# yugabyte/yugabyte-db

Measured on NVIDIA H100. Metric: compaction GB/s (input bytes merged), higher is better.
Workload: dtype u8

## Files before the change

yugabyte-db_b200/csrc/engine.cu:

```cuda
#include "engine.h"
#include "host_sst.h"

#include <cuda_runtime.h>
#include <algorithm>
#include <cstdio>
#include <cstring>
#include <chrono>
#include <cstdlib>
#include <mutex>

namespace ybgpu {

#define CUDA_TRY(expr)                                                                      \
  do {                                                                                      \
    cudaError_t _e = (expr);                                                                \
    if (_e != cudaSuccess) {                                                                \
      return FailCuda(#expr, _e);                                                           \
    }                                                                                       \
  } while (0)

struct RunView {
  const uint8_t* data;
  const uint64_t* blk_off;
  const uint32_t* blk_size;
// ... 423 lines not shown
      const uint8_t* prec = srec - static_cast<size_t>(prm->M) * S;
      inside = rec_ulen(prec, S) >= static_cast<uint32_t>(g) && common_prefix_len(srec, g, prec, g) >= static_cast<uint32_t>(g) &&
               group_prefix_len(prec, rec_ulen(prec, S), prm->R.enabled != 0) == g;
    }
    if (r2 == 0) P.smode[s] = inside ? 1 : 0;
    const RunView& q = P.runs[r2];
    uint32_t lo = 0, hi = q.n_entries;
    if (pass == 1) {
      const uint32_t c0 = s_local - s_local % SAMPLE_COARSE, c1 = c0 + SAMPLE_COARSE;
      lo = P.pos[static_cast<size_t>(P.sample_base[r] + c0) * k + r2];
      if (P.sample_base[r] + c1 < P.sample_base[r + 1]) hi = P.pos[static_cast<size_t>(P.sample_base[r] + c1) * k + r2];
    }
    if (inside) {
      if (r2 == static_cast<uint32_t>(r)) lo = hi = idx;
      while (lo < hi) {
        const uint32_t mid = (lo + hi) >> 1;
        const int c = cmp_records(q.rec + static_cast<size_t>(mid) * S, srec, S);
        if (r2 < static_cast<uint32_t>(r) ? c <= 0 : c < 0) lo = mid + 1; else hi = mid;
      }
    } else {
      while (lo < hi) {
        uint32_t mid = (lo + hi) >> 1;
        const uint8_t* c = q.rec + static_cast<size_t>(mid) * S;
        if (cmp_prefix_vs_key(srec, g, c, rec_ulen(c, S)) > 0) lo = mid + 1; else hi = mid;
      }
    }
    P.pos[static_cast<size_t>(s) * k + r2] = lo;
  }
}

__global__ void __launch_bounds__(256) k_sample_bucket(PartView P, const JobParams* prm) {
  const int k = prm->k;
  for (uint32_t s = blockIdx.x * blockDim.x + threadIdx.x; s < P.n_samples; s += gridDim.x * blockDim.x) {
    unsigned long long rank = 0;
    for (int r = 0; r < k; r++) rank += P.pos[static_cast<size_t>(s) * k + r];
    if (rank == 0) continue;
    uint32_t b = static_cast<uint32_t>(rank / prm->H);
    atomicMin(&P.bucket_min[b], (rank << 28) | s);
  }
}

__device__ __forceinline__ uint32_t block_exclusive_scan(uint32_t v, uint32_t* warp_sums, uint32_t* total) {
  const int lane = threadIdx.x & 31, wid = threadIdx.x >> 5;
  uint32_t x = v;
  for (int o = 1; o < 32; o <<= 1) { uint32_t y = __shfl_up_sync(0xffffffffu, x, o); if (lane >= o) x += y; }
  __syncthreads();
  if (lane == 31) warp_sums[wid] = x;
  __syncthreads();
  if (wid == 0) {
    uint32_t w = lane < (blockDim.x >> 5) ? warp_sums[lane] : 0;
    for (int o = 1; o < 32; o <<= 1) { uint32_t y = __shfl_up_sync(0xffffffffu, w, o); if (lane >= o) w += y; }
    warp_sums[lane] = w;
  }
  __syncthreads();
  uint32_t excl = (wid ? warp_sums[wid - 1] : 0) + x - v;
  if (total) *total = warp_sums[(blockDim.x >> 5) - 1];
  return excl;
}

constexpr int TILE_CHUNK = 2048;
__global__ void __launch_bounds__(256) k_bucket_counts(PartView P, uint32_t* partial) {
  __shared__ uint32_t sh;
  if (threadIdx.x == 0) sh = 0;
  __syncthreads();
  const uint64_t base = static_cast<uint64_t>(blockIdx.x) * TILE_CHUNK;
  uint32_t c = 0;
  for (uint32_t j = threadIdx.x; j < TILE_CHUNK; j += 256) { const uint64_t i = base + j; if (i < P.n_buckets && P.bucket_min[i] != ~0ull) c++; }
  c = __reduce_add_sync(0xffffffffu, c);
  if ((threadIdx.x & 31) == 0 && c) atomicAdd(&sh, c);
  __syncthreads();
  if (threadIdx.x == 0) partial[blockIdx.x] = sh;
}
__global__ void __launch_bounds__(256) k_build_tiles(PartView P, const JobParams* prm, const uint32_t* partial , const uint32_t* total,
                                                     uint32_t* tile_lo, unsigned long long* tile_rank, JobDev* J) {
  __shared__ uint32_t warp_sums[32];
  const int k = prm->k;
  if (blockIdx.x == 0) {
    if (threadIdx.x < k) tile_lo[threadIdx.x] = 0;
    if (threadIdx.x == 0) { tile_rank[0] = 0; J->n_tiles = *total + 1; }
  }
  const uint64_t base = static_cast<uint64_t>(blockIdx.x) * TILE_CHUNK;
  constexpr int PER = TILE_CHUNK / 256;
  unsigned long long v[PER];
  uint32_t c = 0;
  for (int j = 0; j < PER; j++) { const uint64_t i = base + threadIdx.x * PER + j; v[j] = i < P.n_buckets ? P.bucket_min[i] : ~0ull; c += v[j] != ~0ull; }
  uint32_t t = 1 + partial[blockIdx.x] + block_exclusive_scan(c, warp_sums, nullptr);
  for (int j = 0; j < PER; j++) {
    if (v[j] == ~0ull) continue;
    const uint32_t s = static_cast<uint32_t>(v[j] & ((1u << 28) - 1));
    for (int r = 0; r < k; r++) tile_lo[static_cast<size_t>(t) * k + r] = P.pos[static_cast<size_t>(s) * k + r];
    tile_rank[t] = (v[j] >> 28) | (P.smode[s] ? TILE_CONT : 0ull);
    t++;
  }
}

__global__ void __launch_bounds__(256) k_tile_check(const RunView* runs, const uint32_t* tile_lo, int k, JobDev* J) {
  const uint32_t n_tiles = J->n_tiles;
  uint32_t mx = 0;
  for (uint32_t t = blockIdx.x * blockDim.x + threadIdx.x; t < n_tiles; t += gridDim.x * blockDim.x) {
    uint32_t sz = 0;
    for (int r = 0; r < k; r++) {
      const uint32_t lo = tile_lo[static_cast<size_t>(t) * k + r];
      const uint32_t hi = (t + 1 < n_tiles) ? tile_lo[static_cast<size_t>(t + 1) * k + r] : runs[r].n_entries;
      sz += hi - lo;
    }
    mx = max(mx, sz);
  }
  mx = __reduce_max_sync(0xffffffffu, mx);
  if ((threadIdx.x & 31) == 0 && mx) atomicMax(&J->max_tile, mx);
}

struct MergeView {
  const RunView* runs;
  const uint32_t* tile_lo;
  const unsigned long long* tile_rank;
  Desc* desc;
  ValueRewrite* rewrites;
  uint32_t rewrite_cap;
  uint32_t n_tiles;
  uint16_t* fk16;
  uint32_t* fkh;
  int32_t S, k;
  uint32_t cap;
};

constexpr int MERGE_THREADS = 256;
constexpr uint8_t ENT_GROUP_START = 128;
constexpr uint32_t RW_PRE_DROPPED = 0xfffffffeu;
constexpr int RANK_C = 8;
constexpr int RANK_KMAX = 16;

namespace tile_layout {
constexpr uint32_t SEG_LO = 0;
constexpr uint32_t SEG_START = SEG_LO + 4 * MAX_RUNS;
constexpr uint32_t CBASE = SEG_START + 4 * (MAX_RUNS + 2);
constexpr uint32_t CRANK = CBASE + 4 * (MAX_RUNS + 2);
constexpr uint32_t CRANK_FIXED = 2 * (RANK_KMAX + 1) * RANK_KMAX;
constexpr uint32_t CRANK_PER = 2 * RANK_KMAX / RANK_C;
constexpr uint32_t A0 = (CRANK + CRANK_FIXED + 15) & ~15u;
constexpr uint32_t ORDER_K = CRANK_PER;
constexpr uint32_t GLEN_K = ORDER_K + 2;
constexpr uint32_t GSTART_K = GLEN_K + 2;
constexpr uint32_t A1 = A0 + 16;
constexpr uint32_t PVIS_K = GSTART_K + 2;
constexpr uint32_t RES_K = PVIS_K + 2;
constexpr uint32_t RW_K = RES_K + 1;
constexpr uint32_t PFX_K = RW_K + 4;
constexpr uint32_t PFX2_K = PFX_K + 8;
constexpr uint32_t RECS_K = PFX2_K + 8;
static_assert(RANK_KMAX % RANK_C == 0 && (PFX_K % 1) == 0, "layout");
__host__ __device__ constexpr uint32_t bytes(uint32_t S, uint32_t cap) { return A1 + (RECS_K + S + 8) * cap; }
}


static_assert(MAX_RUNS <= REPLAY_MAX_RUNS, "a replay's cursors cover every run of a job");

__device__ __noinline__ int seed_continuation(FeedState* st, const JobParams* prm, const RunView* runs, const uint32_t* seg_lo, int k, int S,
                                              const uint8_t* k0_smem) {
  ReplayRun rr[REPLAY_MAX_RUNS];
  for (int r = 0; r < k; r++) { rr[r].rec = runs[r].rec; rr[r].limit = seg_lo[r]; rr[r].data = runs[r].data; rr[r].val_off = runs[r].val_off; }
  return replay_ancestors(st, prm->R, rr, k, S, k0_smem, rec_ulen(k0_smem, S), prm->bottommost, prm->last_sequence);
}

__device__ __forceinline__ int table_id_len(const uint8_t* e, uint32_t ulen) {
  return (e[0] == 'y' || e[0] == '0') ? dockey_id_size(e, ulen) : 0;
}

__device__ __noinline__ int seed_table_from_runs(Overwrite* ow0, const JobParams* prm, const RunView* runs, const uint32_t* seg_lo,
                                                 const uint32_t* seg_start, int k, int S, const uint8_t* row, int id, bool through_tile) {
  ReplayRun rr[REPLAY_MAX_RUNS];
  for (int r = 0; r < k; r++) {
    rr[r].rec = runs[r].rec; rr[r].data = runs[r].data; rr[r].val_off = runs[r].val_off;
    rr[r].limit = seg_lo[r] + (through_tile ? seg_start[r + 1] - seg_start[r] : 0u);
  }
  FeedState st;
  const int d = replay_table_seed(&st, prm->R, rr, k, S, row, static_cast<uint32_t>(id), prm->bottommost, prm->last_sequence);
  if (d < 0) return d;
  if (!st.n_ow) return 0;
  *ow0 = st.ow[0];
  return 1;
}

__device__ __noinline__ int seed_table_in_tile(FeedState* st, const JobParams* prm, const RunView* runs, const uint8_t* recs, int SS, int S,
                                               const uint16_t* order, const uint32_t* seg_lo, const uint32_t* seg_start,
                                               uint32_t i0, uint32_t i1, const uint8_t* row, int id) {
  feed_state_reset(st);
  const uint8_t* prev = nullptr;
  for (uint32_t i = i0; i < i1; i++) {
    const uint32_t li = order[i];
    const uint8_t* c = recs + static_cast<size_t>(SS) * li;
    if (rec_flags(c, S) & REC_F_HT_FILTERED) continue;
    const uint8_t* val = nullptr;
    if (rec_vlen(c, S) && has_control_fields(rec_vfirst(c, S))) {
      int r = 0;
      while (seg_start[r + 1] <= li) r++;
      val = runs[r].data + runs[r].val_off[seg_lo[r] + (li - seg_start[r])];
    }
    const int d = replay_entry(st, prm->R, c, S, val, &prev, prm->bottommost, prm->last_sequence);
    if (d < 0) return d;
  }
  table_seed(st, row, static_cast<uint32_t>(id));
  return 0;
}

__device__ __forceinline__ uint32_t block_exclusive_max(uint32_t v, uint32_t* warp_sums) {
  const int lane = threadIdx.x & 31, wid = threadIdx.x >> 5;
  uint32_t x = v;
  for (int o = 1; o < 32; o <<= 1) { const uint32_t y = __shfl_up_sync(0xffffffffu, x, o); if (lane >= o) x = max(x, y); }
  uint32_t ex = __shfl_up_sync(0xffffffffu, x, 1);
  if (lane == 0) ex = 0;
  __syncthreads();
  if (lane == 31) warp_sums[wid] = x;
  __syncthreads();
  if (wid == 0) {
    uint32_t m = lane < (blockDim.x >> 5) ? warp_sums[lane] : 0;
    for (int o = 1; o < 32; o <<= 1) { const uint32_t y = __shfl_up_sync(0xffffffffu, m, o); if (lane >= o) m = max(m, y); }
    warp_sums[lane] = m;
  }
  __syncthreads();
  return max(wid ? warp_sums[wid - 1] : 0u, ex);
}

__global__ void __launch_bounds__(MERGE_THREADS, 3) k_merge_filter(MergeView V, const JobParams* prm, JobDev* J) {
  extern __shared__ __align__(16) uint8_t smem[];
  const int S = V.S, k = V.k;
  const int SS = S + 8;
  const uint32_t cap = V.cap;
  namespace L = tile_layout;
  uint32_t* seg_lo = reinterpret_cast<uint32_t*>(smem + L::SEG_LO);
  uint32_t* seg_start = reinterpret_cast<uint32_t*>(smem + L::SEG_START);
  uint32_t* cbase = reinterpret_cast<uint32_t*>(smem + L::CBASE);
  uint16_t* crank = reinterpret_cast<uint16_t*>(smem + L::CRANK);
  uint16_t* order = reinterpret_cast<uint16_t*>(smem + L::A0 + L::ORDER_K * cap);
  uint16_t* glen = reinterpret_cast<uint16_t*>(smem + L::A0 + L::GLEN_K * cap);
  uint16_t* gstart = reinterpret_cast<uint16_t*>(smem + L::A0 + L::GSTART_K * cap);
  uint16_t* pvis = reinterpret_cast<uint16_t*>(smem + L::A1 + L::PVIS_K * cap);
  uint8_t* res = smem + L::A1 + L::RES_K * cap;
  uint32_t* rw_slot = reinterpret_cast<uint32_t*>(smem + L::A1 + L::RW_K * cap);
  unsigned long long* pfx = reinterpret_cast<unsigned long long*>(smem + L::A1 + L::PFX_K * cap);
  unsigned long long* pfx2 = reinterpret_cast<unsigned long long*>(smem + L::A1 + L::PFX2_K * cap);
  uint8_t* recs = smem + L::A1 + L::RECS_K * cap;
  __shared__ uint32_t warp_sums[32];
  __shared__ uint32_t sh_T, sh_ngroups, sh_any_filtered, sh_any_id;
  __shared__ int sh_err;
  __shared__ uint32_t sh_c0;
  __shared__ Overwrite sh_ow0;
  __shared__ int sh_ow0_state;
  __shared__ unsigned long long sh_stats[9];
  __shared__ const uint8_t* sh_pred;
  __shared__ uint32_t sh_rb[2][MAX_RUNS + 2];

  const uint32_t tile = blockIdx.x;
  const bool cont = (V.tile_rank[tile] & TILE_CONT) != 0;
  if (threadIdx.x < 9) sh_stats[threadIdx.x] = 0;
  if (threadIdx.x < 32) {
    static_assert(MAX_RUNS <= 64, "two rounds of 32 lanes cover the runs");
    uint32_t acc = 0;
    for (int r0 = 0; r0 < k; r0 += 32) {
      const int r = r0 + static_cast<int>(threadIdx.x);
      uint32_t lo = 0, n = 0;
      if (r < k) {
        lo = V.tile_lo[static_cast<size_t>(tile) * k + r];
        const uint32_t hi = (tile + 1 < V.n_tiles) ? V.tile_lo[static_cast<size_t>(tile + 1) * k + r] : V.runs[r].n_entries;
        n = hi - lo;
      }
      uint32_t x = n;
      for (int o = 1; o < 32; o <<= 1) { const uint32_t y = __shfl_up_sync(0xffffffffu, x, o); if (static_cast<int>(threadIdx.x) >= o) x += y; }
      if (r < k) { seg_lo[r] = lo; seg_start[r] = acc + x - n; }
      acc += __shfl_sync(0xffffffffu, x, 31);
    }
    if (threadIdx.x == 0) {
      seg_start[k] = acc;
      sh_T = acc;
      sh_any_filtered = 0;
      sh_any_id = 0;
      sh_err = *reinterpret_cast<volatile int*>(&J->error);
    }
  }
  __syncthreads();
  const uint32_t T = sh_T;
  if (T == 0) return;
  if (cont && threadIdx.x == 0) atomicAdd(&J->n_cont_tiles, 1u);
  if (T > cap) { if (threadIdx.x == 0) dev_fail(J, DEV_ERR_TILE_OVERFLOW, tile); return; }

  {
    const uint32_t vpr = S >> 4;
    const uint32_t nvec = T * vpr;
    const bool vpr_pow2 = (vpr & (vpr - 1)) == 0;
    const uint32_t vpr_shift = 31 - __clz(vpr);
#pragma unroll 4
    for (uint32_t i = threadIdx.x; i < nvec; i += blockDim.x) {
      const uint32_t li = vpr_pow2 ? i >> vpr_shift : i / vpr, q = i - li * vpr;
      int r = 0;
      while (seg_start[r + 1] <= li) r++;
      const uint4 v = __ldg(reinterpret_cast<const uint4*>(V.runs[r].rec + static_cast<size_t>(seg_lo[r] + (li - seg_start[r])) * S) + q);
      uint2* d = reinterpret_cast<uint2*>(recs + static_cast<size_t>(li) * SS + 16 * q);
      d[0] = make_uint2(v.x, v.y); d[1] = make_uint2(v.z, v.w);
    }
  }
  __syncthreads();

  if (threadIdx.x < 32) {
    const uint8_t* ref = recs;
    const uint32_t ref_len = rec_ulen(ref, S);
    uint32_t c = 0xffffffffu;
    for (int r = static_cast<int>(threadIdx.x); r < k; r += 32) {
      const uint32_t n = seg_start[r + 1] - seg_start[r];
      if (!n) continue;
      const uint8_t* f = recs + static_cast<size_t>(SS) * seg_start[r];
      const uint8_t* l = recs + static_cast<size_t>(SS) * (seg_start[r + 1] - 1);
      c = min(c, min(common_prefix_len(ref, ref_len, f, rec_ulen(f, S)), common_prefix_len(ref, ref_len, l, rec_ulen(l, S))));
    }
    c = __reduce_min_sync(0xffffffffu, c);
    c = min(c, ref_len) & ~7u;
    if (c + 16 > static_cast<uint32_t>(S - 16)) c = (S - 16 >= 16) ? static_cast<uint32_t>(S - 32) & ~7u : 0;
    if (threadIdx.x == 0) sh_c0 = c;
  }
  if (threadIdx.x == 0) {
    const uint8_t* pred = nullptr;
    if (cont) {
      for (int r = 0; r < k; r++) {
        uint32_t j = seg_lo[r];
        const uint8_t* c2 = nullptr;
        while (j > 0) {
          const uint8_t* q = V.runs[r].rec + static_cast<size_t>(j - 1) * S;
          if (!(rec_flags(q, S) & REC_F_INVISIBLE)) { c2 = q; break; }
          j--;
        }
        if (c2 && (!pred || cmp_records(c2, pred, S) >= 0)) pred = c2;
      }
    }
    sh_pred = pred;
  }
  __syncthreads();
  {
    const uint32_t c0 = sh_c0;
    for (uint32_t li = threadIdx.x; li < T; li += blockDim.x)
    {
      pfx[li] = bswap64(ld_u64_aligned(recs + static_cast<size_t>(SS) * li + c0));
      pfx2[li] = bswap64(ld_u64_aligned(recs + static_cast<size_t>(SS) * li + c0 + 8));
    }
  }
  __syncthreads();

  {
    constexpr int MT = 2;
    uint16_t* bufs[2] = {order, reinterpret_cast<uint16_t*>(crank)};
    auto le = [&](uint32_t a, uint32_t b) -> bool {
      const unsigned long long pa = pfx[a], pb = pfx[b];
      if (pa != pb) return pa < pb;
      const unsigned long long qa = pfx2[a], qb = pfx2[b];
      if (qa != qb) return qa < qb;
      return cmp_records(recs + static_cast<size_t>(SS) * a, recs + static_cast<size_t>(SS) * b, S) <= 0;
    };
    for (uint32_t li = threadIdx.x; li < T; li += blockDim.x) bufs[0][li] = static_cast<uint16_t>(li);
    if (threadIdx.x <= static_cast<uint32_t>(k)) sh_rb[0][threadIdx.x] = seg_start[threadIdx.x];
    __syncthreads();
    int nruns = k, cur = 0;
    while (nruns > 1) {
      const uint16_t* src = bufs[cur]; uint16_t* dst = bufs[cur ^ 1];
      const uint32_t* rb = sh_rb[cur];
      const int npairs = (nruns + 1) >> 1;
      for (uint32_t o0 = threadIdx.x * MT; o0 < T; o0 += blockDim.x * MT) {
        int p = 0;
        while (p + 1 < npairs && rb[2 * (p + 1)] <= o0) p++;
        uint32_t a0 = rb[2 * p], a1 = rb[min(2 * p + 1, nruns)], b1 = rb[min(2 * p + 2, nruns)];
        const uint32_t d = o0 - a0, la = a1 - a0, lb = b1 - a1;
        uint32_t lo = d > lb ? d - lb : 0, hi = min(d, la);
        while (lo < hi) {
          const uint32_t mid = (lo + hi) >> 1;
          if (le(src[a0 + mid], src[a1 + (d - 1 - mid)])) lo = mid + 1; else hi = mid;
        }
        uint32_t i = a0 + lo, j = a1 + (d - lo);
        const uint32_t o_end = min(o0 + MT, T);
        for (uint32_t o = o0; o < o_end; o++) {
          while (o == b1 && p + 1 < npairs) {
            p++;
            a0 = rb[2 * p]; a1 = rb[min(2 * p + 1, nruns)]; b1 = rb[min(2 * p + 2, nruns)];
            i = a0; j = a1;
          }
          uint16_t pick;
          if (i < a1 && (j >= b1 || le(src[i], src[j]))) pick = src[i++]; else pick = src[j++];
          dst[o] = pick;
        }
      }
      if (threadIdx.x <= static_cast<uint32_t>(npairs)) sh_rb[cur ^ 1][threadIdx.x] = rb[min(2 * static_cast<int>(threadIdx.x), nruns)];
      __syncthreads();
      nruns = npairs; cur ^= 1;
    }
    if (cur) {
      for (uint32_t li = threadIdx.x; li < T; li += blockDim.x) order[li] = bufs[1][li];
    }
  }
  for (uint32_t li = threadIdx.x; li < T; li += blockDim.x) {
    int r = 0;
    while (seg_start[r + 1] <= li) r++;
    const uint32_t p = li - seg_start[r];
    const uint8_t* e = recs + static_cast<size_t>(SS) * li;
    if (p > 0 && cmp_records(e - SS, e, S) >= 0) { dev_fail(J, DEV_ERR_UNSORTED, tile); sh_err = 1; }
    int fk = 0;
    const int g = group_prefix_len(e, rec_ulen(e, S), prm->R.enabled != 0, V.fk16 ? &fk : nullptr);
    if (g < 0) { dev_fail(J, -g, tile); sh_err = 1; glen[li] = 0; } else glen[li] = static_cast<uint16_t>(g);
    if (V.fk16) {
      const uint32_t gid = V.runs[r].gid_base + seg_lo[r] + p;
      V.fk16[gid] = static_cast<uint16_t>(g < 0 ? 0 : fk);
      if (V.fkh) V.fkh[gid] = (g < 0 || fk <= 0) ? 0u : leveldb_hash(e, static_cast<uint32_t>(fk), kBloomSeed);
    }
    if (rec_flags(e, S) & REC_F_INVISIBLE) sh_any_filtered = 1;
    if (e[0] == 'y' || e[0] == '0') sh_any_id = 1;
  }
  __syncthreads();
  if (sh_err) return;

  if (sh_any_filtered) {
    if (threadIdx.x == 0) {
      uint32_t last = 0xffff;
      for (uint32_t i = 0; i < T; i++) {
        pvis[i] = static_cast<uint16_t>(last);
        if (!(rec_flags(recs + static_cast<size_t>(SS) * (order[i]), S) & REC_F_INVISIBLE)) last = i;
      }
    }
  } else {
    for (uint32_t i = threadIdx.x; i < T; i += blockDim.x) pvis[i] = static_cast<uint16_t>(i ? i - 1 : 0xffff);
  }
  __syncthreads();

  const uint32_t items = (T + blockDim.x - 1) / blockDim.x;
  uint32_t my_groups = 0;
  unsigned long long st_counted = 0, st_hidden = 0, st_obsolete = 0, st_in_k = 0, st_in_v = 0;
  for (uint32_t j = 0; j < items; j++) {
    const uint32_t i = threadIdx.x * items + j;
    if (i >= T) break;
    const uint32_t li = order[i];
    const uint8_t* e = recs + static_cast<size_t>(SS) * (li);
    uint8_t f = 0;
    if (!(rec_flags(e, S) & REC_F_INVISIBLE)) {
      f |= ENT_COUNTED; st_counted++;
      st_in_k += rec_ulen(e, S) + 8; st_in_v += rec_vlen(e, S);
      const uint64_t suffix = rec_suffix(e, S);
      const uint32_t type = static_cast<uint32_t>(suffix & 0xff);
      const uint64_t seq = suffix >> 8;
      if (type != 0 && type != 1) dev_fail(J, DEV_ERR_UNSUPPORTED_VALUE, tile);
      const uint32_t ulen = rec_ulen(e, S);
      bool first_occ = true;
      if (pvis[i] != 0xffff) {
        const uint8_t* pe = recs + static_cast<size_t>(SS) * (order[pvis[i]]);
        first_occ = cmp_user_keys(pe, rec_ulen(pe, S), e, ulen) != 0;
      } else if (cont && sh_pred) {
        first_occ = cmp_user_keys(sh_pred, rec_ulen(sh_pred, S), e, ulen) != 0;
      }
      if (!first_occ) { f |= ENT_DROP_HIDDEN; st_hidden++; }
      else if (type == 0 && prm->bottommost && seq <= prm->last_sequence) { f |= ENT_DROP_OBSOLETE; st_obsolete++; }
      else {
        f |= ENT_KEEP;
        if (prm->bottommost && seq < prm->last_sequence) {
          bool is_largest = ulen == prm->largest_len;
          for (uint32_t q = 0; is_largest && q < ulen; q++) is_largest = e[q] == prm->largest[q];
          if (!is_largest) f |= ENT_ZERO_SEQ;
        }
      }
    }
    bool gs = i == 0;
    if (!gs) {
      const uint32_t lp = order[i - 1];
      const uint32_t g = glen[li];
      gs = glen[lp] != g || common_prefix_len(e, g, recs + static_cast<size_t>(SS) * (lp), g) < g;
    }
    if (gs) { my_groups++; f |= ENT_GROUP_START; }
    res[i] = f;
  }
  uint32_t ngroups;
  uint32_t gbase = block_exclusive_scan(my_groups, warp_sums, &ngroups);
  for (uint32_t j = 0; j < items; j++) {
    const uint32_t i = threadIdx.x * items + j;
    if (i >= T) break;
    if (res[i] & ENT_GROUP_START) gstart[gbase++] = static_cast<uint16_t>(i);
  }
  if (threadIdx.x == 0) { gstart[ngroups] = static_cast<uint16_t>(T); sh_ngroups = ngroups; }
  __syncthreads();

  unsigned long long st_feed = 0;
  for (uint32_t i = threadIdx.x; i < T; i += blockDim.x) {
    uint32_t mark = 0xffffffffu;
    if (i > 0 && prm->R.enabled && (res[i] & ENT_KEEP) && (res[i - 1] & ENT_KEEP)) {
      const uint8_t* e = recs + static_cast<size_t>(SS) * order[i];
      const uint8_t* p = recs + static_cast<size_t>(SS) * order[i - 1];
      const uint32_t ul = rec_ulen(e, S), pl = rec_ulen(p, S);
      const uint32_t hl = doc_ht_len_from_end(e, ul), hp = doc_ht_len_from_end(p, pl);
      if (hl && hp && ul - hl == pl - hp &&
          !(rec_vlen(e, S) && rec_vfirst(e, S) == 'k') && !(rec_vlen(p, S) && rec_vfirst(p, S) == 'k')) {
        const EncHt& chosen = (e[0] == 'y' && prm->R.has_cotables_cutoff) ? prm->R.cotables_cutoff_enc : prm->R.cutoff_enc;
        if (encht_cmp(p + pl - hp, hp, chosen.b, chosen.n) <= 0 && common_prefix_len(e, ul - hl, p, ul - hl) >= ul - hl)
          mark = RW_PRE_DROPPED;
      }
    }
    rw_slot[i] = mark;
  }
  const bool ids = prm->R.enabled && sh_any_id;
  if (ids) {
    const uint32_t ngroups = sh_ngroups;
    if (threadIdx.x == 0) {
      int state = 0;
      const uint8_t* e = recs + static_cast<size_t>(SS) * order[0];
      const uint32_t ul = rec_ulen(e, S);
      const int id = table_id_len(e, ul);
      if (id > 0 && static_cast<uint32_t>(id) < ul) {
        bool lookup = e[id] != '!';
        if (!lookup && cont && ngroups > 1) {
          const uint8_t* n1 = recs + static_cast<size_t>(SS) * order[gstart[1]];
          lookup = rec_ulen(n1, S) > static_cast<uint32_t>(id) && n1[id] != '!' && common_prefix_len(n1, id, e, id) >= static_cast<uint32_t>(id);
        }
        if (lookup) {
          const int rc = seed_table_from_runs(&sh_ow0, prm, V.runs, seg_lo, seg_start, k, S, e, id, e[id] == '!');
          if (rc < 0) dev_fail(J, -rc, tile);
          state = rc > 0 ? 2 : 1;
        }
      }
      sh_ow0_state = state;
    }
    const uint32_t per = (ngroups + blockDim.x - 1) / blockDim.x;
    const uint32_t g0 = min(threadIdx.x * per, ngroups), g1 = min(g0 + per, ngroups);
    uint32_t last = 0;
    for (uint32_t g = g0; g < g1; g++) {
      bool head = g == 0;
      if (!head) {
        const uint8_t* e = recs + static_cast<size_t>(SS) * order[gstart[g]];
        const uint8_t* p = recs + static_cast<size_t>(SS) * order[gstart[g - 1]];
        const int id = table_id_len(e, rec_ulen(e, S));
        head = id <= 0 || table_id_len(p, rec_ulen(p, S)) != id || common_prefix_len(p, id, e, id) < static_cast<uint32_t>(id);
      }
      if (head) last = g + 1;
      pvis[g] = static_cast<uint16_t>(last ? last - 1 : 0xffff);
    }
    const uint32_t carry = block_exclusive_max(last, warp_sums);
    for (uint32_t g = g0; g < g1 && pvis[g] == 0xffff; g++) pvis[g] = static_cast<uint16_t>(carry - 1);
  }
  __syncthreads();
  if (prm->R.enabled) {
    for (uint32_t g = threadIdx.x; g < sh_ngroups; g += blockDim.x) {
      FeedState st;
      feed_state_reset(&st);
      const uint32_t i0 = gstart[g], i1 = gstart[g + 1];
      if (ids) {
        const uint8_t* e0 = recs + static_cast<size_t>(SS) * order[i0];
        const uint32_t ul0 = rec_ulen(e0, S);
        const int id = table_id_len(e0, ul0);
        if (id > 0 && static_cast<uint32_t>(id) < ul0 && e0[id] != '!') {
          const uint32_t h = pvis[g];
          if (h == 0 && sh_ow0_state) {
            if (sh_ow0_state == 2) feed_state_seed(&st, e0, id, sh_ow0);
          } else if (recs[static_cast<size_t>(SS) * order[gstart[h]] + id] == '!') {
            const int rc = seed_table_in_tile(&st, prm, V.runs, recs, SS, S, order, seg_lo, seg_start, gstart[h], gstart[h + 1], e0, id);
            if (rc < 0) { dev_fail(J, -rc, tile); continue; }
          }
        }
      }
      const bool continued = cont && g == 0;
      if (continued) {
        const int rc = seed_continuation(&st, prm, V.runs, seg_lo, k, S, recs + static_cast<size_t>(SS) * order[i0]);
        if (rc < 0) { dev_fail(J, -rc, tile); continue; }
      }
      {
        bool all_above = !(prm->R.lower_len | prm->R.upper_len) && !continued;
        for (uint32_t i = i0; i < i1 && all_above; i++) {
          if (!(res[i] & ENT_KEEP)) continue;
          const uint8_t* e = recs + static_cast<size_t>(SS) * (order[i]);
          const uint32_t ulen = rec_ulen(e, S);
          const uint8_t b0 = ulen ? e[0] : 10;
          const uint32_t htl = doc_ht_len_from_end(e, ulen);
          const uint8_t vf = rec_vfirst(e, S);
          if (b0 == 10 || b0 == 6 || b0 == 7 || b0 == 'y' || b0 == '0' || !htl ||
              encht_cmp(e + ulen - htl, htl, prm->R.cutoff_enc.b, prm->R.cutoff_enc.n) <= 0 ||
              (rec_vlen(e, S) && (has_control_fields(vf) || vf == 'z' || vf == '|')))
            all_above = false;
        }
        if (all_above) continue;
      }
      for (uint32_t i = i0; i < i1; i++) {
        uint8_t f = res[i];
        if (!(f & ENT_KEEP)) continue;
        if (rw_slot[i] == RW_PRE_DROPPED) { rw_slot[i] = 0xffffffffu; res[i] = f & ~ENT_KEEP & ~ENT_ZERO_SEQ; st_feed++; continue; }
        const uint32_t li = order[i];
        const uint8_t* e = recs + static_cast<size_t>(SS) * (li);
        int r = 0;
        while (seg_start[r + 1] <= li) r++;
        const uint32_t idx = seg_lo[r] + (li - seg_start[r]);
        const uint32_t vlen = rec_vlen(e, S);
        const uint8_t vfirst = rec_vfirst(e, S);
        const uint8_t* val = nullptr;
        if (vlen && has_control_fields(vfirst)) val = V.runs[r].data + V.runs[r].val_off[idx];
        ValueRewrite rw;
        int d = feed_step(&st, prm->R, e, rec_ulen(e, S), vfirst, val, vlen, &rw);
        if (d < 0) { dev_fail(J, -d, tile); break; }
        if (d == 0) { res[i] = f & ~ENT_KEEP & ~ENT_ZERO_SEQ; st_feed++; continue; }
        f |= static_cast<uint8_t>(d);
        if (d & ENT_VAL_REENCODE) {
          uint32_t slot = atomicAdd(&J->n_rewrites, 1u);
          if (slot < V.rewrite_cap) { V.rewrites[slot] = rw; rw_slot[i] = slot; }
          else dev_fail(J, DEV_ERR_UNSUPPORTED_VALUE, tile);
        }
        res[i] = f;
      }
    }
  }
  if (prm->R.enabled) {
    for (uint32_t g = threadIdx.x; g < sh_ngroups; g += blockDim.x) {
      const uint32_t i0 = gstart[g], i1 = gstart[g + 1];
      bool done = false;
      for (uint32_t i = i0; i < i1; i++) {
        uint8_t f = res[i] & static_cast<uint8_t>(~ENT_FIRST_OF_ROW);
        if (!done && (f & ENT_KEEP)) { f |= ENT_FIRST_OF_ROW; done = true; }
        res[i] = f;
      }
    }
  }
  __syncthreads();

  const unsigned long long rank0 = V.tile_rank[tile] & ~TILE_CONT;
  unsigned long long st_kept = 0, st_kbytes = 0, st_vbytes = 0, mn = ~0ull, mx = 0;
  for (uint32_t i = threadIdx.x; i < T; i += blockDim.x) {
    const uint32_t li = order[i];
    const uint8_t* e = recs + static_cast<size_t>(SS) * (li);
    int r = 0;
    while (seg_start[r + 1] <= li) r++;
    const uint32_t idx = seg_lo[r] + (li - seg_start[r]);
    const uint8_t f = res[i];
    Desc d;
    d.gid = V.runs[r].gid_base + idx;
    d.klen = static_cast<uint16_t>(rec_ulen(e, S) + 8);
    d.flags = prm->R.enabled ? f : (f & static_cast<uint8_t>(~ENT_GROUP_START)); d.run = static_cast<uint8_t>(r);
    d.rewrite_slot = rw_slot[i];
    uint32_t vout = rec_vlen(e, S);
    if (f & ENT_VAL_TOMBSTONE) vout = 1;
    else if (f & ENT_VAL_REENCODE) { const ValueRewrite& rw = V.rewrites[rw_slot[i]]; vout = vout - rw.skip + rw.prefix_len; }
    d.vlen_out = vout;
    if ((f & ENT_KEEP) && !(f & ENT_VAL_REENCODE)) {
      uint32_t sh = 0xffffu;
      int j = static_cast<int>(i) - 1;
      for (int steps = 0; j >= 0 && !(res[j] & ENT_KEEP) && steps < 24; steps++) j--;
      if (j >= 0 && (res[j] & ENT_KEEP)) {
        const uint8_t* p = recs + static_cast<size_t>(SS) * order[j];
        const uint32_t m = min(rec_ulen(e, S), rec_ulen(p, S));
        const uint32_t c = common_prefix_len(e, m, p, m);
        if (c < m) sh = c;
      }
      d.rewrite_slot = sh;
    }
    V.desc[rank0 + i] = d;
    if (f & ENT_KEEP) {
      st_kept++; st_kbytes += d.klen; st_vbytes += vout;
      if ((rec_suffix(e, S) & 0xff) != 1) atomicAdd(&J->n_kept_deletions, 1ull);
      const unsigned long long seq = (f & ENT_ZERO_SEQ) ? 0ull : (rec_suffix(e, S) >> 8);
      mn = min(mn, seq); mx = max(mx, seq);
    }
  }
  unsigned long long vals[9] = {st_counted, st_hidden, st_obsolete, st_feed, st_kept, st_kbytes, st_vbytes, st_in_k, st_in_v};
  for (int q = 0; q < 9; q++) {
    unsigned long long v = vals[q];
    if (__any_sync(0xffffffffu, (v >> 26) != 0)) {
      for (int o = 16; o; o >>= 1) v += __shfl_xor_sync(0xffffffffu, v, o);
    } else {
      v = __reduce_add_sync(0xffffffffu, static_cast<unsigned>(v));
    }
    if ((threadIdx.x & 31) == 0 && v) atomicAdd(&sh_stats[q], v);
  }
  for (int o = 16; o; o >>= 1) { mn = min(mn, __shfl_xor_sync(0xffffffffu, mn, o)); mx = max(mx, __shfl_xor_sync(0xffffffffu, mx, o)); }
  if ((threadIdx.x & 31) == 0) { if (mn != ~0ull) atomicMin(&J->min_seq, mn); if (mx) atomicMax(&J->max_seq, mx); }
  __syncthreads();
  if (threadIdx.x == 0) {
    if (sh_stats[0]) atomicAdd(&J->n_counted, sh_stats[0]);
    if (sh_stats[1]) atomicAdd(&J->n_hidden, sh_stats[1]);
    if (sh_stats[2]) atomicAdd(&J->n_obsolete, sh_stats[2]);
    if (sh_stats[3]) atomicAdd(&J->n_feed_dropped, sh_stats[3]);
    if (sh_stats[4]) atomicAdd(&J->n_kept, sh_stats[4]);
    if (sh_stats[5]) atomicAdd(&J->out_key_bytes, sh_stats[5]);
    if (sh_stats[6]) atomicAdd(&J->out_val_bytes, sh_stats[6]);
    if (sh_stats[7]) atomicAdd(&J->in_key_bytes, sh_stats[7]);
    if (sh_stats[8]) atomicAdd(&J->in_val_bytes, sh_stats[8]);
  }
}

constexpr int EMIT_CHUNK = 2048;
constexpr int EMIT_THREADS = 256;

struct Sums3 { unsigned long long n, kb, vb; };

__global__ void __launch_bounds__(EMIT_THREADS) k_emit_sums(const Desc* desc, uint64_t N, Sums3* partial) {
  __shared__ unsigned long long sh[3];
  if (threadIdx.x < 3) sh[threadIdx.x] = 0;
  __syncthreads();
  const uint64_t base = static_cast<uint64_t>(blockIdx.x) * EMIT_CHUNK;
  unsigned long long n = 0, kb = 0, vb = 0;
  for (uint32_t j = threadIdx.x; j < EMIT_CHUNK; j += blockDim.x) {
    uint64_t i = base + j;
    if (i < N) { Desc d = desc[i]; if (d.flags & ENT_KEEP) { n++; kb += d.klen; vb += d.vlen_out; } }
  }
  for (int o = 16; o; o >>= 1) { n += __shfl_xor_sync(0xffffffffu, n, o); kb += __shfl_xor_sync(0xffffffffu, kb, o); vb += __shfl_xor_sync(0xffffffffu, vb, o); }
  if ((threadIdx.x & 31) == 0) { atomicAdd(&sh[0], n); atomicAdd(&sh[1], kb); atomicAdd(&sh[2], vb); }
  __syncthreads();
  if (threadIdx.x == 0) { partial[blockIdx.x].n = sh[0]; partial[blockIdx.x].kb = sh[1]; partial[blockIdx.x].vb = sh[2]; }
}

__global__ void __launch_bounds__(1024) k_scan_sums(Sums3* partial, uint32_t n) {
  __shared__ unsigned long long ws[3][32];
  __shared__ unsigned long long carry[3];
  if (threadIdx.x < 3) carry[threadIdx.x] = 0;
  __syncthreads();
  const int lane = threadIdx.x & 31, wid = threadIdx.x >> 5;
  for (uint32_t base = 0; base < n; base += 1024) {
    uint32_t i = base + threadIdx.x;
    unsigned long long v[3] = {0, 0, 0};
    if (i < n) { v[0] = partial[i].n; v[1] = partial[i].kb; v[2] = partial[i].vb; }
    unsigned long long x[3] = {v[0], v[1], v[2]};
    for (int q = 0; q < 3; q++) {
      for (int o = 1; o < 32; o <<= 1) { unsigned long long y = __shfl_up_sync(0xffffffffu, x[q], o); if (lane >= o) x[q] += y; }
      if (lane == 31) ws[q][wid] = x[q];
    }
    __syncthreads();
    if (wid == 0) {
      for (int q = 0; q < 3; q++) {
        unsigned long long w = ws[q][lane];
        for (int o = 1; o < 32; o <<= 1) { unsigned long long y = __shfl_up_sync(0xffffffffu, w, o); if (lane >= o) w += y; }
        ws[q][lane] = w;
      }
    }
    __syncthreads();
    if (i < n) {
      partial[i].n = carry[0] + (wid ? ws[0][wid - 1] : 0) + x[0] - v[0];
      partial[i].kb = carry[1] + (wid ? ws[1][wid - 1] : 0) + x[1] - v[1];
      partial[i].vb = carry[2] + (wid ? ws[2][wid - 1] : 0) + x[2] - v[2];
    }
    __syncthreads();
    if (threadIdx.x < 3) carry[threadIdx.x] += ws[threadIdx.x][31];
    __syncthreads();
  }
}

__device__ __forceinline__ void warp_copy(uint8_t* dst, const uint8_t* src, uint32_t n, int lane) {
  uint32_t head = (4 - (reinterpret_cast<uintptr_t>(dst) & 3)) & 3;
  if (head > n) head = n;
  if (lane < static_cast<int>(head)) dst[lane] = src[lane];
  dst += head; src += head; n -= head;
  const uint32_t nw = n >> 2;
  const uint32_t sh = reinterpret_cast<uintptr_t>(src) & 3;
  const uint32_t* s32 = reinterpret_cast<const uint32_t*>(src - sh);
  uint32_t* d32 = reinterpret_cast<uint32_t*>(dst);
  for (uint32_t w = lane; w < nw; w += 32) {
    uint32_t lo = __ldg(s32 + w);
    if (sh) { uint32_t hi = __ldg(s32 + w + 1); lo = __funnelshift_r(lo, hi, sh * 8); }
    d32[w] = lo;
  }
  const uint32_t tail = n & 3;
  if (lane < static_cast<int>(tail)) dst[nw * 4 + lane] = src[nw * 4 + lane];
}

struct EmitView {
  const RunView* runs;
  const Desc* desc;
  const Sums3* partial;
  const ValueRewrite* rewrites;
  uint8_t* out_keys; uint64_t* out_koff;
  uint8_t* out_vals; uint64_t* out_voff;
  uint64_t N;
};

__global__ void __launch_bounds__(EMIT_THREADS) k_emit(EmitView E, int S, JobDev* J) {
  __shared__ uint32_t s_n[EMIT_CHUNK + 1];
  __shared__ uint32_t s_kb[EMIT_CHUNK + 1];
  __shared__ uint32_t s_vb[EMIT_CHUNK + 1];
  __shared__ uint32_t warp_sums[32];
  const uint64_t base = static_cast<uint64_t>(blockIdx.x) * EMIT_CHUNK;
  const Sums3 off = E.partial[blockIdx.x];
  constexpr int PER = EMIT_CHUNK / EMIT_THREADS;
  uint32_t n = 0, kb = 0, vb = 0;
  uint32_t ln[PER], lk[PER], lv[PER];
  for (int j = 0; j < PER; j++) {
    uint64_t i = base + threadIdx.x * PER + j;
    ln[j] = n; lk[j] = kb; lv[j] = vb;
    if (i < E.N) { Desc d = E.desc[i]; if (d.flags & ENT_KEEP) { n++; kb += d.klen; vb += d.vlen_out; } }
  }
  uint32_t bn = block_exclusive_scan(n, warp_sums, nullptr);
  uint32_t bk = block_exclusive_scan(kb, warp_sums, nullptr);
  uint32_t bv = block_exclusive_scan(vb, warp_sums, nullptr);
  for (int j = 0; j < PER; j++) {
    uint32_t q = threadIdx.x * PER + j;
    s_n[q] = bn + ln[j]; s_kb[q] = bk + lk[j]; s_vb[q] = bv + lv[j];
  }
  __syncthreads();
  const int lane = threadIdx.x & 31, wid = threadIdx.x >> 5;
  for (uint32_t q = wid; q < EMIT_CHUNK; q += EMIT_THREADS / 32) {
    const uint64_t i = base + q;
    if (i >= E.N) break;
    const Desc d = E.desc[i];
    if (!(d.flags & ENT_KEEP)) continue;
    const RunView& run = E.runs[d.run];
    const uint32_t idx = d.gid - run.gid_base;
    const uint8_t* rec = run.rec + static_cast<size_t>(idx) * S;
    const uint64_t j = off.n + s_n[q];
    const uint64_t ko = off.kb + s_kb[q], vo = off.vb + s_vb[q];
    if (lane == 0) { E.out_koff[j] = ko; E.out_voff[j] = vo; }
    const uint32_t ulen = d.klen - 8u;
    uint8_t* kd = E.out_keys + ko;
    for (uint32_t b = lane; b < ulen; b += 32) kd[b] = rec[b];
    if (lane < 8) {
      uint64_t suffix = rec_suffix(rec, S);
      if (d.flags & ENT_ZERO_SEQ) suffix &= 0xff;
      kd[ulen + lane] = static_cast<uint8_t>(suffix >> (8 * lane));
    }
    uint8_t* vd = E.out_vals + vo;
    const uint8_t* vs = run.data + run.val_off[idx];
    if (d.flags & ENT_VAL_TOMBSTONE) {
      if (lane == 0) vd[0] = 'X';
    } else if (d.flags & ENT_VAL_REENCODE) {
      const ValueRewrite& rw = E.rewrites[d.rewrite_slot];
      if (lane < rw.prefix_len) vd[lane] = rw.prefix[lane];
      const uint32_t rest = d.vlen_out - rw.prefix_len;
      for (uint32_t b = lane; b < rest; b += 32) vd[rw.prefix_len + b] = vs[rw.skip + b];
    } else {
      warp_copy(vd, vs, d.vlen_out, lane);
    }
  }
  (void)J;
}

__device__ __forceinline__ unsigned long long mix64(unsigned long long x) {
  x ^= x >> 33; x *= 0xff51afd7ed558ccdull; x ^= x >> 33; x *= 0xc4ceb9fe1a85ec53ull; x ^= x >> 33; return x;
}
__global__ void __launch_bounds__(256) k_digest(const uint8_t* keys, const uint64_t* koff, const uint8_t* vals,
                                                const uint64_t* voff, uint64_t n, JobDev* J) {
  unsigned long long acc = 0;
  for (uint64_t i = blockIdx.x * static_cast<uint64_t>(blockDim.x) + threadIdx.x; i < n;
// ... 1611 lines not shown
```

Before: 278.3.

## Stage run/index per record, use cp.async loads, and batch block stats reduction

The staging loop now copies records into shared memory with cp.async and stores each record's run and source index in the 8 spare bytes after the record. Later passes (sort check, table seeding, feed, descriptor emit) read these instead of linearly scanning seg_start for the run. The feed loop is moved into a noinline feed_row helper with a row_above_cutoff precheck. Per-warp stats, including kept deletions and min/max seq, are gathered into shared memory and reduced once per block, replacing per-entry global atomics and shared atomics. The cost is extra shared writes per record and a larger, restructured stats reduction that reuses the pfx buffer.

```diff
diff --git a/yugabyte-db_b200/csrc/engine.cu b/yugabyte-db_b200/csrc/engine.cu
--- a/yugabyte-db_b200/csrc/engine.cu
+++ b/yugabyte-db_b200/csrc/engine.cu
@@ -599,6 +599,9 @@
 __host__ __device__ constexpr uint32_t bytes(uint32_t S, uint32_t cap) { return A1 + (RECS_K + S + 8) * cap; }
 }
 
+__device__ __forceinline__ uint32_t staged_run(const uint8_t* rec, int S) { return *reinterpret_cast<const uint32_t*>(rec + S); }
+__device__ __forceinline__ uint32_t staged_idx(const uint8_t* rec, int S) { return *reinterpret_cast<const uint32_t*>(rec + S + 4); }
+
 
 static_assert(MAX_RUNS <= REPLAY_MAX_RUNS, "a replay's cursors cover every run of a job");
 
@@ -629,19 +632,16 @@
 }
 
 __device__ __noinline__ int seed_table_in_tile(FeedState* st, const JobParams* prm, const RunView* runs, const uint8_t* recs, int SS, int S,
-                                               const uint16_t* order, const uint32_t* seg_lo, const uint32_t* seg_start,
-                                               uint32_t i0, uint32_t i1, const uint8_t* row, int id) {
+                                               const uint16_t* order, uint32_t i0, uint32_t i1, const uint8_t* row, int id) {
   feed_state_reset(st);
   const uint8_t* prev = nullptr;
   for (uint32_t i = i0; i < i1; i++) {
-    const uint32_t li = order[i];
-    const uint8_t* c = recs + static_cast<size_t>(SS) * li;
+    const uint8_t* c = recs + static_cast<size_t>(SS) * order[i];
     if (rec_flags(c, S) & REC_F_HT_FILTERED) continue;
     const uint8_t* val = nullptr;
     if (rec_vlen(c, S) && has_control_fields(rec_vfirst(c, S))) {
-      int r = 0;
-      while (seg_start[r + 1] <= li) r++;
-      val = runs[r].data + runs[r].val_off[seg_lo[r] + (li - seg_start[r])];
+      const uint32_t r = staged_run(c, S);
+      val = runs[r].data + runs[r].val_off[staged_idx(c, S)];
     }
     const int d = replay_entry(st, prm->R, c, S, val, &prev, prm->bottommost, prm->last_sequence);
     if (d < 0) return d;
@@ -649,6 +649,75 @@
   table_seed(st, row, static_cast<uint32_t>(id));
   return 0;
 }
+
+__device__ __forceinline__ bool row_above_cutoff(const JobParams* prm, const uint8_t* recs, int SS, int S, const uint16_t* order,
+                                                 const uint8_t* res, uint32_t i0, uint32_t i1) {
+  if (prm->R.lower_len | prm->R.upper_len) return false;
+  for (uint32_t i = i0; i < i1; i++) {
+    if (!(res[i] & ENT_KEEP)) continue;
+    const uint8_t* e = recs + static_cast<size_t>(SS) * (order[i]);
+    const uint32_t ulen = rec_ulen(e, S);
+    const uint8_t b0 = ulen ? e[0] : 10;
+    const uint32_t htl = doc_ht_len_from_end(e, ulen);
+    const uint8_t vf = rec_vfirst(e, S);
+    if (b0 == 10 || b0 == 6 || b0 == 7 || b0 == 'y' || b0 == '0' || !htl ||
+        encht_cmp(e + ulen - htl, htl, prm->R.cutoff_enc.b, prm->R.cutoff_enc.n) <= 0 ||
+        (rec_vlen(e, S) && (has_control_fields(vf) || vf == 'z' || vf == '|')))
+      return false;
+  }
+  return true;
+}
+
+__device__ __noinline__ uint32_t feed_row(const JobParams* prm, JobDev* J, const RunView* runs, ValueRewrite* rewrites, uint32_t rewrite_cap,
+                                          const uint32_t* seg_lo, int k, const uint8_t* recs, int SS, int S, const uint16_t* order,
+                                          const uint16_t* gstart, const uint16_t* blk, uint8_t* res, uint32_t* rw_slot, uint32_t g, int id,
+                                          bool continued, int ow0_state, const Overwrite* ow0, uint32_t tile) {
+  FeedState st;
+  feed_state_reset(&st);
+  const uint32_t i0 = gstart[g], i1 = gstart[g + 1];
+  if (id > 0) {
+    const uint8_t* e0 = recs + static_cast<size_t>(SS) * order[i0];
+    const uint32_t h = blk[g];
+    if (h == 0 && ow0_state) {
+      if (ow0_state == 2) feed_state_seed(&st, e0, id, *ow0);
+    } else if (recs[static_cast<size_t>(SS) * order[gstart[h]] + id] == '!') {
+      const int rc = seed_table_in_tile(&st, prm, runs, recs, SS, S, order, gstart[h], gstart[h + 1], e0, id);
+      if (rc < 0) { dev_fail(J, -rc, tile); return 0; }
+    }
+  }
+  if (continued) {
+    const int rc = seed_continuation(&st, prm, runs, seg_lo, k, S, recs + static_cast<size_t>(SS) * order[i0]);
+    if (rc < 0) { dev_fail(J, -rc, tile); return 0; }
+  }
+  uint32_t dropped = 0;
+  for (uint32_t i = i0; i < i1; i++) {
+    uint8_t f = res[i];
+    if (!(f & ENT_KEEP)) continue;
+    if (rw_slot[i] == RW_PRE_DROPPED) { rw_slot[i] = 0xffffffffu; res[i] = f & ~ENT_KEEP & ~ENT_ZERO_SEQ; dropped++; continue; }
+    const uint8_t* e = recs + static_cast<size_t>(SS) * order[i];
+    const uint32_t vlen = rec_vlen(e, S);
+    const uint8_t vfirst = rec_vfirst(e, S);
+    const uint8_t* val = nullptr;
+    if (vlen && has_control_fields(vfirst)) { const uint32_t r = staged_run(e, S); val = runs[r].data + runs[r].val_off[staged_idx(e, S)]; }
+    ValueRewrite rw;
+    int d = feed_step(&st, prm->R, e, rec_ulen(e, S), vfirst, val, vlen, &rw);
+    if (d < 0) { dev_fail(J, -d, tile); break; }
+    if (d == 0) { res[i] = f & ~ENT_KEEP & ~ENT_ZERO_SEQ; dropped++; continue; }
+    f |= static_cast<uint8_t>(d);
+    if (d & ENT_VAL_REENCODE) {
+      uint32_t slot = atomicAdd(&J->n_rewrites, 1u);
+      if (slot < rewrite_cap) { rewrites[slot] = rw; rw_slot[i] = slot; }
+      else dev_fail(J, DEV_ERR_UNSUPPORTED_VALUE, tile);
+    }
+    res[i] = f;
+  }
+  return dropped;
+}
+
+__device__ __forceinline__ void cp_async_8(void* dst, const void* src) {
+  asm volatile("cp.async.ca.shared.global [%0], [%1], 8;" ::"r"(static_cast<uint32_t>(__cvta_generic_to_shared(dst))), "l"(src) : "memory");
+}
+__device__ __forceinline__ void cp_async_wait_all() { asm volatile("cp.async.wait_all;" ::: "memory"); }
 
 __device__ __forceinline__ uint32_t block_exclusive_max(uint32_t v, uint32_t* warp_sums) {
   const int lane = threadIdx.x & 31, wid = threadIdx.x >> 5;
@@ -693,13 +762,11 @@
   __shared__ uint32_t sh_c0;
   __shared__ Overwrite sh_ow0;
   __shared__ int sh_ow0_state;
-  __shared__ unsigned long long sh_stats[9];
   __shared__ const uint8_t* sh_pred;
   __shared__ uint32_t sh_rb[2][MAX_RUNS + 2];
 
   const uint32_t tile = blockIdx.x;
   const bool cont = (V.tile_rank[tile] & TILE_CONT) != 0;
-  if (threadIdx.x < 9) sh_stats[threadIdx.x] = 0;
   if (threadIdx.x < 32) {
     static_assert(MAX_RUNS <= 64, "two rounds of 32 lanes cover the runs");
     uint32_t acc = 0;
@@ -735,15 +802,19 @@
     const uint32_t nvec = T * vpr;
     const bool vpr_pow2 = (vpr & (vpr - 1)) == 0;
     const uint32_t vpr_shift = 31 - __clz(vpr);
+    int r = 0;
 #pragma unroll 4
     for (uint32_t i = threadIdx.x; i < nvec; i += blockDim.x) {
       const uint32_t li = vpr_pow2 ? i >> vpr_shift : i / vpr, q = i - li * vpr;
-      int r = 0;
       while (seg_start[r + 1] <= li) r++;
-      const uint4 v = __ldg(reinterpret_cast<const uint4*>(V.runs[r].rec + static_cast<size_t>(seg_lo[r] + (li - seg_start[r])) * S) + q);
-      uint2* d = reinterpret_cast<uint2*>(recs + static_cast<size_t>(li) * SS + 16 * q);
-      d[0] = make_uint2(v.x, v.y); d[1] = make_uint2(v.z, v.w);
-    }
+      const uint32_t idx = seg_lo[r] + (li - seg_start[r]);
+      const uint8_t* src = V.runs[r].rec + static_cast<size_t>(idx) * S + 16 * q;
+      uint8_t* dst = recs + static_cast<size_t>(li) * SS + 16 * q;
+      cp_async_8(dst, src);
+      cp_async_8(dst + 8, src + 8);
+      if (q == 0) *reinterpret_cast<uint2*>(recs + static_cast<size_t>(li) * SS + S) = make_uint2(static_cast<uint32_t>(r), idx);
+    }
+    cp_async_wait_all();
   }
   __syncthreads();
 
@@ -840,16 +911,14 @@
     }
   }
   for (uint32_t li = threadIdx.x; li < T; li += blockDim.x) {
-    int r = 0;
-    while (seg_start[r + 1] <= li) r++;
-    const uint32_t p = li - seg_start[r];
     const uint8_t* e = recs + static_cast<size_t>(SS) * li;
-    if (p > 0 && cmp_records(e - SS, e, S) >= 0) { dev_fail(J, DEV_ERR_UNSORTED, tile); sh_err = 1; }
+    const uint32_t r = staged_run(e, S);
+    if (li > seg_start[r] && cmp_records(e - SS, e, S) >= 0) { dev_fail(J, DEV_ERR_UNSORTED, tile); sh_err = 1; }
     int fk = 0;
     const int g = group_prefix_len(e, rec_ulen(e, S), prm->R.enabled != 0, V.fk16 ? &fk : nullptr);
     if (g < 0) { dev_fail(J, -g, tile); sh_err = 1; glen[li] = 0; } else glen[li] = static_cast<uint16_t>(g);
     if (V.fk16) {
-      const uint32_t gid = V.runs[r].gid_base + seg_lo[r] + p;
+      const uint32_t gid = V.runs[r].gid_base + staged_idx(e, S);
       V.fk16[gid] = static_cast<uint16_t>(g < 0 ? 0 : fk);
       if (V.fkh) V.fkh[gid] = (g < 0 || fk <= 0) ? 0u : leveldb_hash(e, static_cast<uint32_t>(fk), kBloomSeed);
     }
@@ -985,69 +1054,18 @@
   __syncthreads();
   if (prm->R.enabled) {
     for (uint32_t g = threadIdx.x; g < sh_ngroups; g += blockDim.x) {
-      FeedState st;
-      feed_state_reset(&st);
       const uint32_t i0 = gstart[g], i1 = gstart[g + 1];
+      int id = 0;
       if (ids) {
         const uint8_t* e0 = recs + static_cast<size_t>(SS) * order[i0];
         const uint32_t ul0 = rec_ulen(e0, S);
-        const int id = table_id_len(e0, ul0);
-        if (id > 0 && static_cast<uint32_t>(id) < ul0 && e0[id] != '!') {
-          const uint32_t h = pvis[g];
-          if (h == 0 && sh_ow0_state) {
-            if (sh_ow0_state == 2) feed_state_seed(&st, e0, id, sh_ow0);
-          } else if (recs[static_cast<size_t>(SS) * order[gstart[h]] + id] == '!') {
-            const int rc = seed_table_in_tile(&st, prm, V.runs, recs, SS, S, order, seg_lo, seg_start, gstart[h], gstart[h + 1], e0, id);
-            if (rc < 0) { dev_fail(J, -rc, tile); continue; }
-          }
-        }
+        id = table_id_len(e0, ul0);
+        if (id <= 0 || static_cast<uint32_t>(id) >= ul0 || e0[id] == '!') id = 0;
       }
       const bool continued = cont && g == 0;
-      if (continued) {
-        const int rc = seed_continuation(&st, prm, V.runs, seg_lo, k, S, recs + static_cast<size_t>(SS) * order[i0]);
-        if (rc < 0) { dev_fail(J, -rc, tile); continue; }
-      }
-      {
-        bool all_above = !(prm->R.lower_len | prm->R.upper_len) && !continued;
-        for (uint32_t i = i0; i < i1 && all_above; i++) {
-          if (!(res[i] & ENT_KEEP)) continue;
-          const uint8_t* e = recs + static_cast<size_t>(SS) * (order[i]);
-          const uint32_t ulen = rec_ulen(e, S);
-          const uint8_t b0 = ulen ? e[0] : 10;
-          const uint32_t htl = doc_ht_len_from_end(e, ulen);
-          const uint8_t vf = rec_vfirst(e, S);
-          if (b0 == 10 || b0 == 6 || b0 == 7 || b0 == 'y' || b0 == '0' || !htl ||
-              encht_cmp(e + ulen - htl, htl, prm->R.cutoff_enc.b, prm->R.cutoff_enc.n) <= 0 ||
-              (rec_vlen(e, S) && (has_control_fields(vf) || vf == 'z' || vf == '|')))
-            all_above = false;
-        }
-        if (all_above) continue;
-      }
-      for (uint32_t i = i0; i < i1; i++) {
-        uint8_t f = res[i];
-        if (!(f & ENT_KEEP)) continue;
-        if (rw_slot[i] == RW_PRE_DROPPED) { rw_slot[i] = 0xffffffffu; res[i] = f & ~ENT_KEEP & ~ENT_ZERO_SEQ; st_feed++; continue; }
-        const uint32_t li = order[i];
-        const uint8_t* e = recs + static_cast<size_t>(SS) * (li);
-        int r = 0;
-        while (seg_start[r + 1] <= li) r++;
-        const uint32_t idx = seg_lo[r] + (li - seg_start[r]);
-        const uint32_t vlen = rec_vlen(e, S);
-        const uint8_t vfirst = rec_vfirst(e, S);
-        const uint8_t* val = nullptr;
-        if (vlen && has_control_fields(vfirst)) val = V.runs[r].data + V.runs[r].val_off[idx];
-        ValueRewrite rw;
-        int d = feed_step(&st, prm->R, e, rec_ulen(e, S), vfirst, val, vlen, &rw);
-        if (d < 0) { dev_fail(J, -d, tile); break; }
-        if (d == 0) { res[i] = f & ~ENT_KEEP & ~ENT_ZERO_SEQ; st_feed++; continue; }
-        f |= static_cast<uint8_t>(d);
-        if (d & ENT_VAL_REENCODE) {
-          uint32_t slot = atomicAdd(&J->n_rewrites, 1u);
-          if (slot < V.rewrite_cap) { V.rewrites[slot] = rw; rw_slot[i] = slot; }
-          else dev_fail(J, DEV_ERR_UNSUPPORTED_VALUE, tile);
-        }
-        res[i] = f;
-      }
+      if (!continued && !id && row_above_cutoff(prm, recs, SS, S, order, res, i0, i1)) continue;
+      st_feed += feed_row(prm, J, V.runs, V.rewrites, V.rewrite_cap, seg_lo, k, recs, SS, S, order, gstart, pvis, res, rw_slot,
+                          g, id, continued, sh_ow0_state, &sh_ow0, tile);
     }
   }
   if (prm->R.enabled) {
@@ -1064,16 +1082,13 @@
   __syncthreads();
 
   const unsigned long long rank0 = V.tile_rank[tile] & ~TILE_CONT;
-  unsigned long long st_kept = 0, st_kbytes = 0, st_vbytes = 0, mn = ~0ull, mx = 0;
+  unsigned long long st_kept = 0, st_kbytes = 0, st_vbytes = 0, st_kdel = 0, mn = ~0ull, mx = 0;
   for (uint32_t i = threadIdx.x; i < T; i += blockDim.x) {
-    const uint32_t li = order[i];
-    const uint8_t* e = recs + static_cast<size_t>(SS) * (li);
-    int r = 0;
-    while (seg_start[r + 1] <= li) r++;
-    const uint32_t idx = seg_lo[r] + (li - seg_start[r]);
+    const uint8_t* e = recs + static_cast<size_t>(SS) * order[i];
+    const uint32_t r = staged_run(e, S);
     const uint8_t f = res[i];
     Desc d;
-    d.gid = V.runs[r].gid_base + idx;
+    d.gid = V.runs[r].gid_base + staged_idx(e, S);
     d.klen = static_cast<uint16_t>(rec_ulen(e, S) + 8);
     d.flags = prm->R.enabled ? f : (f & static_cast<uint8_t>(~ENT_GROUP_START)); d.run = static_cast<uint8_t>(r);
     d.rewrite_slot = rw_slot[i];
@@ -1096,34 +1111,55 @@
     V.desc[rank0 + i] = d;
     if (f & ENT_KEEP) {
       st_kept++; st_kbytes += d.klen; st_vbytes += vout;
-      if ((rec_suffix(e, S) & 0xff) != 1) atomicAdd(&J->n_kept_deletions, 1ull);
+      if ((rec_suffix(e, S) & 0xff) != 1) st_kdel++;
       const unsigned long long seq = (f & ENT_ZERO_SEQ) ? 0ull : (rec_suffix(e, S) >> 8);
       mn = min(mn, seq); mx = max(mx, seq);
     }
   }
-  unsigned long long vals[9] = {st_counted, st_hidden, st_obsolete, st_feed, st_kept, st_kbytes, st_vbytes, st_in_k, st_in_v};
-  for (int q = 0; q < 9; q++) {
-    unsigned long long v = vals[q];
-    if (__any_sync(0xffffffffu, (v >> 26) != 0)) {
-      for (int o = 16; o; o >>= 1) v += __shfl_xor_sync(0xffffffffu, v, o);
-    } else {
-      v = __reduce_add_sync(0xffffffffu, static_cast<unsigned>(v));
-    }
-    if ((threadIdx.x & 31) == 0 && v) atomicAdd(&sh_stats[q], v);
-  }
-  for (int o = 16; o; o >>= 1) { mn = min(mn, __shfl_xor_sync(0xffffffffu, mn, o)); mx = max(mx, __shfl_xor_sync(0xffffffffu, mx, o)); }
-  if ((threadIdx.x & 31) == 0) { if (mn != ~0ull) atomicMin(&J->min_seq, mn); if (mx) atomicMax(&J->max_seq, mx); }
+  constexpr int NSTAT = 12, NWARPS = MERGE_THREADS / 32;
+  unsigned long long vals[NSTAT] = {st_counted, st_hidden, st_obsolete, st_feed, st_kept, st_kbytes, st_vbytes, st_in_k, st_in_v, st_kdel, mn, mx};
+  unsigned long long any_big = 0;
+#pragma unroll
+  for (int q = 0; q < 10; q++) any_big |= vals[q] >> 26;
+  if (__any_sync(0xffffffffu, any_big != 0)) {
+#pragma unroll
+    for (int q = 0; q < 10; q++)
+      for (int o = 16; o; o >>= 1) vals[q] += __shfl_xor_sync(0xffffffffu, vals[q], o);
+  } else {
+#pragma unroll
+    for (int q = 0; q < 10; q++) vals[q] = __reduce_add_sync(0xffffffffu, static_cast<unsigned>(vals[q]));
+  }
+  for (int o = 16; o; o >>= 1) {
+    vals[10] = min(vals[10], __shfl_xor_sync(0xffffffffu, vals[10], o));
+    vals[11] = max(vals[11], __shfl_xor_sync(0xffffffffu, vals[11], o));
+  }
+  unsigned long long* part = pfx;
+  if ((threadIdx.x & 31) == 0) {
+#pragma unroll
+    for (int q = 0; q < NSTAT; q++) part[(threadIdx.x >> 5) * NSTAT + q] = vals[q];
+  }
   __syncthreads();
-  if (threadIdx.x == 0) {
-    if (sh_stats[0]) atomicAdd(&J->n_counted, sh_stats[0]);
-    if (sh_stats[1]) atomicAdd(&J->n_hidden, sh_stats[1]);
-    if (sh_stats[2]) atomicAdd(&J->n_obsolete, sh_stats[2]);
-    if (sh_stats[3]) atomicAdd(&J->n_feed_dropped, sh_stats[3]);
-    if (sh_stats[4]) atomicAdd(&J->n_kept, sh_stats[4]);
-    if (sh_stats[5]) atomicAdd(&J->out_key_bytes, sh_stats[5]);
-    if (sh_stats[6]) atomicAdd(&J->out_val_bytes, sh_stats[6]);
-    if (sh_stats[7]) atomicAdd(&J->in_key_bytes, sh_stats[7]);
-    if (sh_stats[8]) atomicAdd(&J->in_val_bytes, sh_stats[8]);
+  if (threadIdx.x < NSTAT) {
+    const int q = static_cast<int>(threadIdx.x);
+    unsigned long long v = part[q];
+    for (int w = 1; w < NWARPS; w++) {
+      const unsigned long long x = part[w * NSTAT + q];
+      v = q == 10 ? min(v, x) : q == 11 ? max(v, x) : v + x;
+    }
+    switch (q) {
+      case 0: if (v) atomicAdd(&J->n_counted, v); break;
+      case 1: if (v) atomicAdd(&J->n_hidden, v); break;
+      case 2: if (v) atomicAdd(&J->n_obsolete, v); break;
+      case 3: if (v) atomicAdd(&J->n_feed_dropped, v); break;
+      case 4: if (v) atomicAdd(&J->n_kept, v); break;
+      case 5: if (v) atomicAdd(&J->out_key_bytes, v); break;
+      case 6: if (v) atomicAdd(&J->out_val_bytes, v); break;
+      case 7: if (v) atomicAdd(&J->in_key_bytes, v); break;
+      case 8: if (v) atomicAdd(&J->in_val_bytes, v); break;
+      case 9: if (v) atomicAdd(&J->n_kept_deletions, v); break;
+      case 10: if (v != ~0ull) atomicMin(&J->min_seq, v); break;
+      default: if (v) atomicMax(&J->max_seq, v); break;
+    }
   }
 }
 
```

New measurement: 291.0, median of 6. +4.6%, better.
